# arloan/OpticalImageProcessor

Hardware: AMD Instinct MI355X
Metric: Mpix/s end-to-end RRC+stitch on 30000x100000x4 strip; % HBM roofline (higher is better)
Workload: dtype u16 rasters; fp64 RRC/maps, f32 bicubic and FFT; 1 GPU; default action (--do-rrc4pan): PAN 30000x100000 + MSS 4x(7500x25000) per GPU; RRC + 5x10x4 inter-band phase correlations (16000x3000 FFT) + polyfit + bicubic align to 16UC4; width=30000, pan_lines_per_gpu=100000, parallelism=rowblock1, backend=rccl, inputs=resident in HBM

## Files before the change

### opticalimageprocessor_amd/csrc/phasecorr.hip

```cpp
#include "oip_corrgeom.h"
#include "oip_fft.h"
#include "oip_fft_dev.h"
#include "oip_internal.h"

#include <cfloat>
#include <cmath>

namespace {

constexpr int kBlock = 256;

__global__ __launch_bounds__(kBlock) void window_u16_to_f32_kernel(const uint16_t *__restrict__ img, size_t pitch,
                                                                   long row0, int col0, int rows, int cols,
                                                                   float *__restrict__ out)
{
    long i = (long)blockIdx.x * kBlock + threadIdx.x;
    const long n = (long)rows * cols;
    const long stride = (long)gridDim.x * kBlock;
    for (; i < n; i += stride) {
        long y = i / cols;
        int x = (int)(i - y * cols);
        out[i] = (float)img[(size_t)(row0 + y) * pitch + col0 + x];
    }
}
// ... 298 lines not shown
    commit(threadIdx.x);
    long s1 = n1, s2 = n2;
    __syncthreads();
    for (; ky <= half; ky += gridDim.x) {
        int tid = threadIdx.x;
        asm volatile("" : "+v"(tid));
        const bool pair = s1 != s2;
        const int kn = ky + gridDim.x;
        const bool more = kn <= half;
        if (more) {
            n1 = (long)ypos[kn] * P;
            n2 = (long)ypos[M - kn] * P;
            fetch(tid);
        }
        __builtin_amdgcn_sched_barrier(0);
        row_stages<ALL, F, NT, NARR, Rs...>(buf, tw, tid);
#pragma unroll 1
        for (int it = 0; it < NIT; ++it) {
            const int kx = tid + it * NT;
            if (kx >= N) continue;
            const int nkx = kx ? N - kx : 0;
            const bool edge_col = (kx == 0) || (2 * kx == N);
            const bool real_bin = edge_col && (ky == 0 || 2 * ky == M);
            const float2 zk0 = buf[2 * kx], zm0 = buf[2 * nkx + 1];
            const float2 A = spec_of(0, zk0, zm0);
            float2 y0, y0m, y1 = make_float2(0.f, 0.f), y1m = make_float2(0.f, 0.f);
            {
                const float2 C = cross_power_bin_fast(A, spec_of(1, zk0, zm0), real_bin, edge_col);
                y0 = C;
                y0m = make_float2(C.x, -C.y);
            }
            if (NARR == 3) {
                const float2 zk1 = buf[2 * F + 2 * kx], zm1 = buf[2 * F + 2 * nkx + 1];
                const float2 zk2 = buf[4 * F + 2 * kx], zm2 = buf[4 * F + 2 * nkx + 1];
                float2 C = cross_power_bin_fast(A, spec_of(0, zk1, zm1), real_bin, edge_col);
                y0.x -= C.y; y0.y += C.x; y0m.x += C.y; y0m.y += C.x;
                C = cross_power_bin_fast(A, spec_of(1, zk1, zm1), real_bin, edge_col);
                y1 = C;
                y1m = make_float2(C.x, -C.y);
                const float2 B3 = fj.last_part ? spec_of(1, zk2, zm2) : spec_of(0, zk2, zm2);
                C = cross_power_bin_fast(A, B3, real_bin, edge_col);
                y1.x -= C.y; y1.y += C.x; y1m.x += C.y; y1m.y += C.x;
            }
            buf[2 * kx] = make_float2(y0.x, -y0.y);
            buf[2 * nkx + 1] = pair ? make_float2(y0m.x, -y0m.y) : make_float2(0.f, 0.f);
            if (NOUT == 2) {
                buf[2 * F + 2 * kx] = make_float2(y1.x, -y1.y);
                buf[2 * F + 2 * nkx + 1] = pair ? make_float2(y1m.x, -y1m.y) : make_float2(0.f, 0.f);
            }
        }
        __syncthreads();
        asm volatile("" : "+v"(tid));
        row_stages<ALL, F, NT, NOUT, Rs...>(buf, tw, tid);
        if (!ALL && NOUT == 1) __syncthreads();
        float4 ya[NOUT][NIT2], yb[NOUT][NIT2];
#pragma unroll
        for (int o = 0; o < NOUT; ++o) {
#pragma unroll
            for (int it = 0; it < NIT2; ++it) {
                const int q = tid + it * NT;
                if (q < N / 2) {
                    const float4 u = buf4[o * F + 2 * q], v = buf4[o * F + 2 * q + 1];
                    ya[o][it] = make_float4(u.x, -u.y, v.x, -v.y);
                    yb[o][it] = make_float4(u.z, -u.w, v.z, -v.w);
                }
            }
        }
        __syncthreads();
        if (more) commit(tid);
        __builtin_amdgcn_sched_barrier(0);
        const long o1 = s1, o2 = s2;
        s1 = n1; s2 = n2;
#pragma unroll
        for (int o = 0; o < NOUT; ++o) {
            float2 *out = fj.out[o];
#pragma unroll
            for (int it = 0; it < NIT2; ++it) {
                const int q = tid + it * NT;
                if (q < N / 2) {
                    *reinterpret_cast<float4 *>(out + o1 + 2 * q) = ya[o][it];
                    if (pair) *reinterpret_cast<float4 *>(out + o2 + 2 * q) = yb[o][it];
                }
            }
        }
        __syncthreads();
    }
}

struct UpRowsJob {
    const float2 *zp;
    const float2 *zn;
    long zn_stride;
    int Pn;
    float2 *out[4];
    const float2 *xtab;
    int nout;
    const float2 *vtab;
    const uint2 *raw16;
    const int *ypos_s;
    int m;
    float *bound;
    int win_hi, win_lo;
};

__device__ __forceinline__ float2 cmulj(float2 a, float2 b)
{
    oipfft::oip_v2f t, r;
    asm("v_pk_mul_f32 %0, %1, %2 op_sel_hi:[0,1]" : "=v"(t) : "v"(oipfft::to_v(a)), "v"(oipfft::to_v(b)));
    asm("v_pk_fma_f32 %0, %1, %2, %3 op_sel:[1,1,0] op_sel_hi:[1,0,1] neg_hi:[1,0,0]" : "=v"(r) : "v"(oipfft::to_v(a)), "v"(oipfft::to_v(b)), "v"(t));
    return oipfft::to_f2(r);
}
__device__ __forceinline__ float2 cfma(float2 a, float2 b, float2 acc)
{
    oipfft::oip_v2f t, r;
    asm("v_pk_fma_f32 %0, %1, %2, %3 op_sel_hi:[0,1,1]" : "=v"(t) : "v"(oipfft::to_v(a)), "v"(oipfft::to_v(b)), "v"(oipfft::to_v(acc)));
    asm("v_pk_fma_f32 %0, %1, %2, %3 op_sel:[1,1,0] op_sel_hi:[1,0,1] neg_lo:[1,0,0]" : "=v"(r) : "v"(oipfft::to_v(a)), "v"(oipfft::to_v(b)), "v"(t));
    return oipfft::to_f2(r);
}
__device__ __forceinline__ float2 cfmaj(float2 a, float2 b, float2 acc)
{
    oipfft::oip_v2f t, r;
    asm("v_pk_fma_f32 %0, %1, %2, %3 op_sel_hi:[0,1,1]" : "=v"(t) : "v"(oipfft::to_v(a)), "v"(oipfft::to_v(b)), "v"(oipfft::to_v(acc)));
    asm("v_pk_fma_f32 %0, %1, %2, %3 op_sel:[1,1,0] op_sel_hi:[1,0,1] neg_hi:[1,0,0]" : "=v"(r) : "v"(oipfft::to_v(a)), "v"(oipfft::to_v(b)), "v"(t));
    return oipfft::to_f2(r);
}

__device__ __forceinline__ float2 spec2_of(int part, float2 zk, float2 zm)
{
    if (part == 0) return make_float2(zk.x + zm.x, zk.y - zm.y);
    return make_float2(zk.y + zm.y, zm.x - zk.x);
}
__device__ __forceinline__ float2 sfma(float s, float2 v, float2 acc)
{
    OIP_FFT_FMA
    return make_float2(acc.x + s * v.x, acc.y + s * v.y);
}

template <int NT, bool VEXP, bool WIN>
__global__ __launch_bounds__(NT) void corr_rows_up_kernel(UpRowsJob fj, int M, int P, const int *__restrict__ ypos,
                                                          const float2 *__restrict__ twF, const float2 *__restrict__ twS)
{
    constexpr int F = 3000, S = F / 4;
    constexpr int TWF = oipfft::TwTable<F, 25, 15, 8>::value(), TWS = oipfft::TwTable<S, 25, 15, 2>::value();
    constexpr int NB = (F / 2 + 1 + NT - 1) / NT;
    __shared__ __align__(16) float2 buf[2 * 2 * F + 4 * 2 * S];
    __shared__ float2 tw[TWF], tws[TWS];
    __shared__ float2 edge[4][2][4];
    __shared__ float2 edgeA[2][2];
    __shared__ float2 edgeT[2][5];
    float2 *bufN = buf + 4 * F;
    float4 *buf4 = reinterpret_cast<float4 *>(buf), *buf4N = reinterpret_cast<float4 *>(bufN);
    const int half = M / 2;
    int ky = blockIdx.x;
    if (ky > half) return;
    for (int i = threadIdx.x; i < TWF; i += NT) tw[i] = twF[i];
    for (int i = threadIdx.x; i < TWS; i += NT) tws[i] = twS[i];
    if (threadIdx.x < 10) edgeT[threadIdx.x / 5][threadIdx.x % 5] = fj.xtab[(threadIdx.x % 5) * F + (threadIdx.x / 5) * (F / 2)];
    float2 H[NB], G[NB][4];
    auto load_tables = [&](int tid) {
#pragma unroll
        for (int r = 0; r < NB; ++r) {
            int kx = tid + NT * r;
            kx = kx <= F / 2 ? kx : 0;
            H[r] = fj.xtab[kx];
#pragma unroll
            for (int j = 0; j < 4; ++j) G[r][j] = fj.xtab[(1 + j) * F + kx];
        }
    };
    constexpr int NIT2 = (F / 2 + NT - 1) / NT;
    constexpr int NQ = 4 * (S / 2);
    constexpr int NITN = (NQ + NT - 1) / NT;
    float4 la[NIT2], lb[NIT2], na[NITN], nb[NITN];
    long n1 = ypos[ky], n2 = ypos[ky ? M - ky : 0];
    auto narrow_row = [&](int k, long full) { return VEXP ? (long)fj.ypos_s[k % fj.m] : full; };
    long m1 = narrow_row(ky, n1), m2 = narrow_row(ky ? M - ky : 0, n2);
    int kyc = ky;
    float2 vt[5];
    uint2 rawreg[NITN][4];
    auto fetch_narrow = [&](int tid) {
        if (VEXP) {
#pragma unroll
            for (int r = 0; r < 5; ++r) vt[r] = fj.vtab[r * M + kyc];
#pragma unroll
            for (int it = 0; it < NITN; ++it) {
                int q = tid + it * NT;
                q = q < NQ ? q : NQ - 1;
#pragma unroll
                for (int r = 0; r < 4; ++r) rawreg[it][r] = fj.raw16[(long)r * NQ + q];
            }
        }
#pragma unroll
        for (int it = 0; it < NITN; ++it) {
            int q = tid + it * NT;
            q = q < NQ ? q : NQ - 1;
            const int a = q / (S / 2), i = q - a * (S / 2);
            const float2 *z = fj.zn + a * fj.zn_stride + 2 * i;
            na[it] = *reinterpret_cast<const float4 *>(z + m1 * fj.Pn);
            nb[it] = *reinterpret_cast<const float4 *>(z + m2 * fj.Pn);
        }
    };
    auto fetch = [&](int tid) {
#pragma unroll
        for (int it = 0; it < NIT2; ++it) {
            int q = tid + it * NT;
            q = q < F / 2 ? q : F / 2 - 1;
            la[it] = *reinterpret_cast<const float4 *>(fj.zp + n1 * P + 2 * q);
            lb[it] = *reinterpret_cast<const float4 *>(fj.zp + n2 * P + 2 * q);
        }
        if (!VEXP) fetch_narrow(tid);
    };
    auto commit = [&](int tid) {
        if (VEXP) fetch_narrow(tid);
#pragma unroll
        for (int it = 0; it < NIT2; ++it) line_pair_commit<F>(buf4, 0, la[it], lb[it], tid + it * NT);
#pragma unroll
        for (int it = 0; it < NITN; ++it) {
            const int q = tid + it * NT;
            if (q < NQ) {
                const int a = q / (S / 2), i = q - a * (S / 2);
                if (VEXP) {
                    const float2 hv = vt[0];
                    float2 x0 = oipfft::cmul(hv, make_float2(na[it].x, na[it].y)), x1 = oipfft::cmul(hv, make_float2(na[it].z, na[it].w));
                    float2 y0 = cmulj(hv, make_float2(nb[it].x, nb[it].y)), y1 = cmulj(hv, make_float2(nb[it].z, nb[it].w));
#pragma unroll
                    for (int r = 0; r < 4; ++r) {
                        const float2 gv = vt[1 + r];
                        const uint2 u = rawreg[it][r];
                        const float2 w0 = make_float2((float)(u.x & 0xffffu), (float)(u.x >> 16)), w1 = make_float2((float)(u.y & 0xffffu), (float)(u.y >> 16));
                        x0 = cfma(gv, w0, x0); x1 = cfma(gv, w1, x1);
                        y0 = cfmaj(gv, w0, y0); y1 = cfmaj(gv, w1, y1);
                    }
                    na[it] = make_float4(x0.x, x0.y, x1.x, x1.y);
                    nb[it] = make_float4(y0.x, y0.y, y1.x, y1.y);
                }
                buf4N[a * S + 2 * i] = make_float4(na[it].x, na[it].y, nb[it].x, nb[it].y);
                buf4N[a * S + 2 * i + 1] = make_float4(na[it].z, na[it].w, nb[it].z, nb[it].w);
                if (i == 0 || i == S / 2 - 1) {
                    const int j = i ? 2 : 0;
                    edge[a][0][j] = make_float2(na[it].x, na[it].y); edge[a][0][j + 1] = make_float2(na[it].z, na[it].w);
                    edge[a][1][j] = make_float2(nb[it].x, nb[it].y); edge[a][1][j + 1] = make_float2(nb[it].z, nb[it].w);
                }
            }
        }
    };
    fetch(threadIdx.x);
    commit(threadIdx.x);
    long s1 = n1, s2 = n2;
    __syncthreads();
    bool first = true;
    char *const brow = reinterpret_cast<char *>(fj.bound + (long)blockIdx.x * 4 * P);
    for (; ky <= half; ky += gridDim.x) {
        int tid = threadIdx.x;
        asm volatile("" : "+v"(tid));
        const bool pair = s1 != s2;
        const int kn = ky + gridDim.x;
        const bool more = kn <= half;
        if (first) load_tables(tid);
        first = false;
        __builtin_amdgcn_sched_barrier(0);
        oipfft::StagesDual3<F, 1, S, 4, NT, 25, 15, 8, 2>::run(buf, tw, bufN, tws, tid);
        float2 Aa[2 * NB], Ab[2 * NB];
#pragma unroll
        for (int r = 0; r < NB; ++r) {
            const int kx = tid + NT * r, nkx = kx ? F - kx : 0;
            if (kx <= F / 2) {
                const float2 zk = buf[2 * kx], zm = buf[2 * nkx + 1];
                Aa[2 * r] = spec_of(0, zk, zm);
                Ab[2 * r] = spec_of(1, zk, zm);
                const float2 zk2 = buf[2 * nkx], zm2 = buf[2 * kx + 1];
                Aa[2 * r + 1] = spec_of(0, zk2, zm2);
                Ab[2 * r + 1] = spec_of(1, zk2, zm2);
                if (kx == 0 || 2 * kx == F) { edgeA[kx ? 1 : 0][0] = Aa[2 * r]; edgeA[kx ? 1 : 0][1] = Ab[2 * r]; }
            }
        }
        auto xround = [&](int o0, const float2 (&A)[2 * NB]) {
#pragma unroll
            for (int h = 0; h < 2; ++h) {
                const float2 *zn = bufN + (o0 + h) * 2 * S;
                float2 e0[4], e1[4];
#pragma unroll
                for (int j = 0; j < 4; ++j) { e0[j] = edge[o0 + h][0][j]; e1[j] = edge[o0 + h][1][j]; }
                float2 *ob = buf + h * 2 * F;
#pragma unroll
                for (int r = 0; r < NB; ++r) {
                    const int kx = tid + NT * r, nkx = kx ? F - kx : 0;
                    if (kx > F / 2) continue;
                    const int c = kx % S, cm = c ? S - c : 0;
                    float2 S0 = make_float2(0.f, 0.f), T0 = S0, S1 = S0, T1 = S0;
#pragma unroll
                    for (int j = 0; j < 4; ++j) {
                        S0 = sfma(G[r][j].x, e0[j], S0); T0 = sfma(G[r][j].y, e0[j], T0);
                        S1 = sfma(G[r][j].x, e1[j], S1); T1 = sfma(G[r][j].y, e1[j], T1);
                    }
                    {
                        const float2 Z0 = oipfft::csub_rot(oipfft::cadd(oipfft::cmul(H[r], zn[2 * c]), S0), T0);
                        const float2 Z1 = oipfft::cadd_rot(oipfft::cadd(cmulj(H[r], zn[2 * cm + 1]), S1), T1);
                        const float2 C1 = cross_power_bin_fast(A[2 * r], spec2_of(0, Z0, Z1), false, false);
                        const float2 C2 = cross_power_bin_fast(A[2 * r], spec2_of(1, Z0, Z1), false, false);
                        ob[2 * kx] = make_float2(C1.x - C2.y, -(C1.y + C2.x));
                        ob[2 * nkx + 1] = pair ? make_float2(C1.x + C2.y, -(C2.x - C1.y)) : make_float2(0.f, 0.f);
                    }
                    if (kx != 0 && 2 * kx != F) {
                        const float2 Z0 = oipfft::cadd_rot(oipfft::cadd(cmulj(H[r], zn[2 * cm]), S0), T0);
                        const float2 Z1 = oipfft::csub_rot(oipfft::cadd(oipfft::cmul(H[r], zn[2 * c + 1]), S1), T1);
                        const float2 C1 = cross_power_bin_fast(A[2 * r + 1], spec2_of(0, Z0, Z1), false, false);
                        const float2 C2 = cross_power_bin_fast(A[2 * r + 1], spec2_of(1, Z0, Z1), false, false);
                        ob[2 * nkx] = make_float2(C1.x - C2.y, -(C1.y + C2.x));
                        ob[2 * kx + 1] = pair ? make_float2(C1.x + C2.y, -(C2.x - C1.y)) : make_float2(0.f, 0.f);
                    }
                    __builtin_amdgcn_sched_barrier(0);
                }
            }
#pragma unroll 1
            for (int r = 0; r < NB; ++r) {
                const int kx = tid + NT * r;
                if (kx != 0 && 2 * kx != F) continue;
                const bool real_bin = ky == 0 || 2 * ky == M;
                const float2 Ae = edgeA[kx ? 1 : 0][o0 ? 1 : 0];
                float2 He = edgeT[kx ? 1 : 0][0], Ge[4];
#pragma unroll
                for (int j = 0; j < 4; ++j) Ge[j] = edgeT[kx ? 1 : 0][1 + j];
#pragma unroll 1
                for (int h = 0; h < 2; ++h) {
                    const float2 *zn = bufN + (o0 + h) * 2 * S;
                    float2 Z0 = oipfft::cmul(He, zn[0]), Z1 = cmulj(He, zn[1]);
#pragma unroll
                    for (int j = 0; j < 4; ++j) { Z0 = cfma(Ge[j], edge[o0 + h][0][j], Z0); Z1 = cfmaj(Ge[j], edge[o0 + h][1][j], Z1); }
                    const float2 C1 = cross_power_bin(Ae, spec2_of(0, Z0, Z1), real_bin, true);
                    const float2 C2 = cross_power_bin(Ae, spec2_of(1, Z0, Z1), real_bin, true);
                    float2 *ob = buf + h * 2 * F;
                    ob[2 * kx] = make_float2(C1.x - C2.y, -(C1.y + C2.x));
                    ob[2 * kx + 1] = pair ? make_float2(C1.x + C2.y, -(C2.x - C1.y)) : make_float2(0.f, 0.f);
                }
            }
        };
        float4 ya[2][NIT2], yb[2][NIT2];
        auto finish = [&]() {
            __syncthreads();
            asm volatile("" : "+v"(tid));
            oipfft::StagesAll<F, NT, 2, 1, 25, 15, 8>::run(buf, tw, tid);
#pragma unroll
            for (int o = 0; o < 2; ++o) {
#pragma unroll
                for (int it = 0; it < NIT2; ++it) line_pair_read_conj<F>(ya[o][it], yb[o][it], buf4, o * F, tid + it * NT);
            }
            __syncthreads();
        };
        auto store = [&](int o0) {
#pragma unroll
            for (int o = 0; o < 2; ++o) {
                float2 *out = fj.out[o0 + o];
#pragma unroll
                for (int it = 0; it < NIT2; ++it) {
                    const int q = tid + it * NT;
                    if (!WIN || q < fj.win_hi || q >= fj.win_lo) line_pair_store<F>(out, s1 * P, s2 * P, pair, ya[o][it], yb[o][it], q);
                }
            }
        };
        auto bound_add = [&](int o0) {
            int tb = tid;
            asm volatile("" : "+v"(tb));
#pragma unroll
            for (int o = 0; o < 2; ++o) {
#pragma unroll
                for (int it = 0; it < NIT2; ++it) {
                    const int q = tb + it * NT;
                    if (q < F / 2) {
                        const float4 a = ya[o][it], b = yb[o][it];
                        float2 s = make_float2(fabsf(a.x) + fabsf(a.y), fabsf(a.z) + fabsf(a.w));
                        if (pair) { s.x += fabsf(b.x) + fabsf(b.y); s.y += fabsf(b.z) + fabsf(b.w); }
                        float *bp = reinterpret_cast<float *>(brow + (unsigned)((o0 + o) * P + 2 * q) * 4u);
                        unsafeAtomicAdd(bp, s.x);
                        unsafeAtomicAdd(bp + 1, s.y);
                    }
                }
            }
        };
        xround(0, Aa);
        finish();
        if (fj.nout == 4) load_tables(tid);
        __builtin_amdgcn_sched_barrier(0);
        store(0);
        __builtin_amdgcn_sched_barrier(0);
        bound_add(0);
        if (fj.nout == 4) xround(2, Ab);
        __builtin_amdgcn_sched_barrier(0);
        if (more) {
            n1 = oip_sload_i32(ypos, kn);
            n2 = oip_sload_i32(ypos, M - kn);
            m1 = VEXP ? (long)oip_sload_i32(fj.ypos_s, kn % fj.m) : n1;
            m2 = VEXP ? (long)oip_sload_i32(fj.ypos_s, (M - kn) % fj.m) : n2;
            kyc = kn;
            fetch(tid);
        }
        __builtin_amdgcn_sched_barrier(0);
        if (fj.nout == 4) finish();
        if (more) commit(tid);
        __builtin_amdgcn_sched_barrier(0);
        if (more) load_tables(tid);
        __builtin_amdgcn_sched_barrier(0);
        if (fj.nout == 4) {
            store(2);
            __builtin_amdgcn_sched_barrier(0);
            bound_add(2);
        }
        s1 = n1; s2 = n2;
        __syncthreads();
    }
}

struct VRowsJob {
    const float2 *zp;
    const float2 *zn;
    long zn_stride;
    int Pn;
    float2 *out[4];
    int nout;
    const float2 *vtab;
    const float2 *raw;
    const int *ypos_s;
    int m;
};

template <int F, int NT, int... Rs>
__global__ __launch_bounds__(NT, 2 * NT / 256) void corr_rows_v_kernel(VRowsJob fj, int a0, int part, int M, int P, const int *__restrict__ ypos,
                                                                      const float2 *__restrict__ twF)
{
    constexpr int TWN = oipfft::TwTable<F, Rs...>::value();
    constexpr int N = F, NARR = 3, NB = 2;
    constexpr int NIT = (N + NT - 1) / NT;
    static_assert(N % 2 == 0, "two points per lane");
    constexpr int NIT2 = (N / 2 + NT - 1) / NT;
    constexpr int NQ = NB * (N / 2);
    constexpr int NITN = (NQ + NT - 1) / NT;
    __shared__ __align__(16) float2 buf[NARR * 2 * F];
    __shared__ float2 tw[TWN];
    float4 *buf4 = reinterpret_cast<float4 *>(buf);
    const int half = M / 2;
    int ky = blockIdx.x;
    if (ky > half) return;
    for (int i = threadIdx.x; i < TWN; i += NT) tw[i] = twF[i];
    float4 la[NIT2], lb[NIT2], na[NITN], nb[NITN];
    float2 vt[5];
    long n1 = ypos[ky], n2 = ypos[ky ? M - ky : 0];
    long m1 = fj.ypos_s[ky % fj.m], m2 = fj.ypos_s[(ky ? M - ky : 0) % fj.m];
    int kyc = ky;
    const float2 *zn = fj.zn + (long)a0 * fj.zn_stride;
    const float2 *raw = fj.raw + (long)a0 * fj.zn_stride;
    auto fetch = [&](int tid) {
#pragma unroll
        for (int it = 0; it < NIT2; ++it) {
            int q = tid + it * NT;
            q = q < N / 2 ? q : N / 2 - 1;
            la[it] = *reinterpret_cast<const float4 *>(fj.zp + n1 * P + 2 * q);
            lb[it] = *reinterpret_cast<const float4 *>(fj.zp + n2 * P + 2 * q);
        }
#pragma unroll
        for (int it = 0; it < NITN; ++it) {
            int q = tid + it * NT;
            q = q < NQ ? q : NQ - 1;
            const int a = q / (N / 2), i = q - a * (N / 2);
            const float2 *z = zn + a * fj.zn_stride + 2 * i;
            na[it] = *reinterpret_cast<const float4 *>(z + m1 * fj.Pn);
            nb[it] = *reinterpret_cast<const float4 *>(z + m2 * fj.Pn);
        }
#pragma unroll
        for (int r = 0; r < 5; ++r) vt[r] = fj.vtab[r * M + kyc];
    };
    auto commit = [&](int tid) {
#pragma unroll
        for (int it = 0; it < NIT2; ++it) line_pair_commit<N>(buf4, 0, la[it], lb[it], tid + it * NT);
#pragma unroll
        for (int it = 0; it < NITN; ++it) {
            const int q = tid + it * NT;
            if (q >= NQ) continue;
            const int a = q / (N / 2), i = q - a * (N / 2);
            const float2 hv = vt[0];
            float2 x0 = oipfft::cmul(hv, make_float2(na[it].x, na[it].y)), x1 = oipfft::cmul(hv, make_float2(na[it].z, na[it].w));
            float2 y0 = cmulj(hv, make_float2(nb[it].x, nb[it].y)), y1 = cmulj(hv, make_float2(nb[it].z, nb[it].w));
#pragma unroll
            for (int r = 0; r < 4; ++r) {
                const float4 rw = *reinterpret_cast<const float4 *>(raw + ((long)r * 4 + a) * fj.zn_stride + 2 * i);
                const float2 gv = vt[1 + r];
                const float2 w0 = make_float2(rw.x, rw.y), w1 = make_float2(rw.z, rw.w);
                x0 = cfma(gv, w0, x0); x1 = cfma(gv, w1, x1);
                y0 = cfmaj(gv, w0, y0); y1 = cfmaj(gv, w1, y1);
            }
            buf4[(1 + a) * F + 2 * i] = make_float4(x0.x, x0.y, y0.x, y0.y);
            buf4[(1 + a) * F + 2 * i + 1] = make_float4(x1.x, x1.y, y1.x, y1.y);
        }
    };
    fetch(threadIdx.x);
    commit(threadIdx.x);
    long s1 = n1, s2 = n2;
    __syncthreads();
    for (; ky <= half; ky += gridDim.x) {
        int tid = threadIdx.x;
        asm volatile("" : "+v"(tid));
        const bool pair = s1 != s2;
        const int kn = ky + gridDim.x;
        const bool more = kn <= half;
        if (more) {
            n1 = ypos[kn];
            n2 = ypos[M - kn];
            m1 = fj.ypos_s[kn % fj.m];
            m2 = fj.ypos_s[(M - kn) % fj.m];
            kyc = kn;
            fetch(tid);
        }
        __builtin_amdgcn_sched_barrier(0);
        oipfft::StagesPipe<F, NT, NARR, 1, Rs...>::run(buf, tw, tid);
#pragma unroll 1
        for (int it = 0; it < NIT; ++it) {
            const int kx = tid + it * NT;
            if (kx >= N) continue;
            const int nkx = kx ? N - kx : 0;
            const bool edge_col = (kx == 0) || (2 * kx == N);
            const bool real_bin = edge_col && (ky == 0 || 2 * ky == M);
            const float2 A = spec_of(part, buf[2 * kx], buf[2 * nkx + 1]);
#pragma unroll
            for (int a = 0; a < NB; ++a) {
                float2 *b = buf + (1 + a) * 2 * F;
                const float2 zk = b[2 * kx], zm = b[2 * nkx + 1];
                const float2 C1 = cross_power_bin_fast(A, spec_of(0, zk, zm), real_bin, edge_col);
                const float2 C2 = cross_power_bin_fast(A, spec_of(1, zk, zm), real_bin, edge_col);
                b[2 * kx] = make_float2(C1.x - C2.y, -(C1.y + C2.x));
                b[2 * nkx + 1] = pair ? make_float2(C1.x + C2.y, -(C2.x - C1.y)) : make_float2(0.f, 0.f);
            }
        }
        __syncthreads();
        asm volatile("" : "+v"(tid));
        oipfft::StagesPipe<F, NT, NB, 1, Rs...>::run(buf + 2 * F, tw, tid);
        float4 ya[NB][NIT2], yb[NB][NIT2];
#pragma unroll
        for (int o = 0; o < NB; ++o) {
#pragma unroll
            for (int it = 0; it < NIT2; ++it) line_pair_read_conj<N>(ya[o][it], yb[o][it], buf4, (1 + o) * F, tid + it * NT);
        }
        __syncthreads();
        if (more) commit(tid);
        __builtin_amdgcn_sched_barrier(0);
#pragma unroll
        for (int o = 0; o < NB; ++o) {
            float2 *out = fj.out[a0 + o];
#pragma unroll
            for (int it = 0; it < NIT2; ++it) line_pair_store<N>(out, s1 * P, s2 * P, pair, ya[o][it], yb[o][it], tid + it * NT);
        }
        s1 = n1; s2 = n2;
        __syncthreads();
    }
}

struct HPackJob {
    const uint16_t *bx[4], *by[4];
    long pitch[4];
};
__global__ __launch_bounds__(128) void hpack_bands_kernel(HPackJob job, int m, int n, int cols, int stride, int Pn, const int *__restrict__ xofs,
                                                          const float4 *__restrict__ alpha, float2 *__restrict__ z, float2 *__restrict__ raw)
{
    const int x = blockIdx.x * 128 + threadIdx.x;
    const int a = blockIdx.z;
// ... 685 lines not shown
    double *const res[1] = {d_result};
    return peak_windows(ctx, pl, w, y, res, 1, 1);
}

int correlate_four(oip_ctx *ctx, const OipFft2dPlan *pl, const PcWork &w, const FusedRow *rk, float2 *zp, float2 *zq,
                   float2 *zl, int last_part, double *d_results )
{
    const SpecRef sa[4] = {{zp, 0}, {zp, 0}, {zp, 0}, {zp, 0}};
    const SpecRef sb[4] = {{zp, 1}, {zq, 0}, {zq, 1}, {zl, last_part}};
    float2 *const y[2] = {w.y[0], w.y[1]};
    int rc;
    if ((rc = xpower_stage(ctx, pl, rk, sa, sb, 4, y))) return rc;
    if ((rc = inverse_to_slots(ctx, pl, w, w.y[0], rk != nullptr, 0))) return rc;
    if ((rc = inverse_to_slots(ctx, pl, w, w.y[1], rk != nullptr, 1))) return rc;
    double *const res[2] = {d_results, d_results + 6};
    return peak_windows(ctx, pl, w, y, res, 2, 2);
}

int correlate_one_to_four(oip_ctx *ctx, const OipFft2dPlan *pl, const PcWork &w, RealSrc a, const RealSrc b[4],
                          int rows, int cols, double *d_results , const HTaps *vt)
{
    const FusedRow *rk = row_stage(pl);
    const bool skip = rk != nullptr;
    int rc;
    if ((rc = forward_packed(ctx, pl, w.z[0], a, b[0], rows, cols, skip, vt))) return rc;
    if ((rc = forward_packed(ctx, pl, w.z[1], b[1], b[2], rows, cols, skip, vt))) return rc;
    if ((rc = forward_packed(ctx, pl, w.z[2], b[3], src_none(), rows, cols, skip, vt))) return rc;
    return correlate_four(ctx, pl, w, rk, w.z[0], w.z[1], w.z[2], 0, d_results);
}

int correlate_two_units(oip_ctx *ctx, const OipFft2dPlan *pl, const PcWork &w, RealSrc aA, const RealSrc bA[4], RealSrc aB,
                        const RealSrc bB[4], int rows, int cols, double *d_resA , double *d_resB, const HTaps *vt)
{
    const FusedRow *rk = row_stage(pl);
    const bool skip = rk != nullptr;
    int rc;
    if ((rc = forward_packed(ctx, pl, w.z[0], aA, bA[0], rows, cols, skip, vt))) return rc;
    if ((rc = forward_packed(ctx, pl, w.z[1], bA[1], bA[2], rows, cols, skip, vt))) return rc;
    if ((rc = forward_packed(ctx, pl, w.z[2], aB, bB[0], rows, cols, skip, vt))) return rc;
    if ((rc = forward_packed(ctx, pl, w.z[3], bB[1], bB[2], rows, cols, skip, vt))) return rc;
    if ((rc = forward_packed(ctx, pl, w.z[4], bA[3], bB[3], rows, cols, skip, vt))) return rc;
    if ((rc = correlate_four(ctx, pl, w, rk, w.z[0], w.z[1], w.z[4], 0, d_resA))) return rc;
    return correlate_four(ctx, pl, w, rk, w.z[2], w.z[3], w.z[4], 1, d_resB);
}

struct IbUnit {
    const uint16_t *pan;
    long pan_pitch;
    const uint16_t *band[OIP_MSS_BANDS];
    long band_pitch;
};

struct UpPath {
    const OipFft2dPlan *narrow;
    const OipFft2dPlan *small;
    const float2 *xtab, *vtab;
    bool vonly;
};

struct BandPackJob {
    const uint16_t *bx[4], *by[4];
    long pitch[4];
};
template <bool PAIRS>
__global__ __launch_bounds__(128) void pack_bands_kernel(BandPackJob job, int m, int n, int Pn, float2 *__restrict__ z, unsigned *__restrict__ raw16)
{
    constexpr int W = PAIRS ? 2 : 1;
    const int p = W * (blockIdx.x * 128 + threadIdx.x);
    const int a = blockIdx.z;
    if (p >= n) return;
    const uint16_t *bx = job.bx[a] + p, *by = job.by[a] + p;
    const long pitch = job.pitch[a];
#pragma unroll 4
    for (int y = blockIdx.y; y < m; y += gridDim.y) {
        const int r = y < 2 ? y : (y >= m - 2 ? y - (m - 4) : -1);
        if (PAIRS) {
            const unsigned ux = *reinterpret_cast<const unsigned *>(bx + y * pitch), uy = *reinterpret_cast<const unsigned *>(by + y * pitch);
            *reinterpret_cast<float4 *>(z + (long)y * Pn + a * n + p) =
                make_float4((float)(ux & 0xffffu), (float)(uy & 0xffffu), (float)(ux >> 16), (float)(uy >> 16));
            if (r >= 0) *reinterpret_cast<uint2 *>(raw16 + ((long)r * 4 + a) * n + p) = make_uint2((ux & 0xffffu) | (uy << 16), (ux >> 16) | (uy & 0xffff0000u));
        } else {
            const unsigned ux = bx[y * pitch], uy = by[y * pitch];
            z[(long)y * Pn + a * n + p] = make_float2((float)ux, (float)uy);
            if (r >= 0) raw16[((long)r * 4 + a) * n + p] = ux | (uy << 16);
        }
    }
}

int correlate_units_up(oip_ctx *ctx, const OipFft2dPlan *pl, const UpPath &up, const PcWork &w, RealSrc aA, RealSrc aB, const RealSrc *v ,
                       const IbUnit *const *units, int nunits, int rows, int cols, int band_rows, int band_cols, double *d_resA, double *d_resB,
                       int win_r = -1, int *d_miss = nullptr)
{
    int rc;
    if ((rc = forward_packed(ctx, pl, w.z[0], aA, nunits > 1 ? aB : src_none(), rows, cols, true))) return rc;
    const int narr = 2 * nunits;
    long zn_stride;
    int Pn;
    const int *ypos_s = nullptr;
    unsigned *raw = nullptr;
    if (up.vtab) {
        Pn = up.small->P;
        zn_stride = band_cols;
        raw = reinterpret_cast<unsigned *>(w.z[1] + (long)up.small->M * Pn);
        BandPackJob bj;
        for (int a = 0; a < 4; ++a) {
            const IbUnit *u = units[(a < narr ? a : 0) / 2];
            bj.bx[a] = u->band[2 * (a & 1)]; bj.by[a] = u->band[2 * (a & 1) + 1]; bj.pitch[a] = u->band_pitch;
        }
        {
            OipProfScope prof(ctx, "pack_bands_kernel");
            bool pairs = (band_cols & 1) == 0 && (Pn & 1) == 0;
            for (int a = 0; a < 4; ++a)
                pairs = pairs && (bj.pitch[a] & 1) == 0 && ((size_t)bj.bx[a] & 3) == 0 && ((size_t)bj.by[a] & 3) == 0;
            const int gy = band_rows < 128 ? band_rows : 128;
            if (pairs)
                hipLaunchKernelGGL(pack_bands_kernel<true>, dim3((band_cols / 2 + 127) / 128, gy, 4), dim3(128), 0, ctx->stream, bj, band_rows, band_cols, Pn,
                                   w.z[1], raw);
            else
                hipLaunchKernelGGL(pack_bands_kernel<false>, dim3((band_cols + 127) / 128, gy, 4), dim3(128), 0, ctx->stream, bj, band_rows, band_cols, Pn,
                                   w.z[1], raw);
            OIP_HIP(ctx, hipGetLastError());
        }
        ctx->prof_tag = "_band";
        rc = oip_fft2d_exec(ctx, up.small, w.z[1], 0, nullptr, 1);
        ctx->prof_tag = nullptr;
        if (rc) return rc;
        ypos_s = up.small->d_ypos;
    } else {
        Pn = up.narrow->P;
        zn_stride = (long)up.narrow->M * Pn;
        ctx->prof_tag = "_quarter";
        for (int a = 0; a < narr && !rc; ++a)
            rc = forward_packed(ctx, up.narrow, w.z[1] + a * zn_stride, src_f32(v[2 * a].v), src_f32(v[2 * a + 1].v), rows, band_cols, true);
        ctx->prof_tag = nullptr;
        if (rc) return rc;
    }
    const float2 *twF, *twS;
    if ((rc = oip_fft_table(ctx, 3000, &twF)) || (rc = oip_fft_table(ctx, 750, &twS))) return rc;
    UpRowsJob fj;
    memset(&fj, 0, sizeof fj);
    fj.zp = w.z[0];
    fj.zn = w.z[1];
    fj.zn_stride = zn_stride;
    fj.Pn = Pn;
    for (int o = 0; o < 4; ++o) fj.out[o] = w.y[o];
    fj.xtab = up.xtab;
    fj.nout = narr;
    fj.vtab = up.vtab;
    fj.raw16 = reinterpret_cast<const uint2 *>(raw);
    fj.ypos_s = ypos_s;
    fj.m = band_rows;
    fj.bound = w.prune.bound;
    if (!fj.bound) return oip_fail(ctx, OIP_E_RUNTIME, "correlate_units_up: no storage for the column bounds");
    OIP_HIP(ctx, hipMemsetAsync(fj.bound, 0, sizeof(float) * (size_t)w.prune.groups * 4 * pl->P, ctx->stream));
    PruneWork pw = w.prune;
    const char *pe = getenv("OIP_PEAK_PRUNE");
    const int full = pe && atoi(pe) == 0 ? 1 : 0;
    if (full || !up.vtab || !rows_window_fits(pw, win_r) || !d_miss) win_r = -1;
    pw.win_r = win_r;
    pw.miss = d_miss;
    if (win_r >= 0) {
        fj.win_hi = ((win_r + 1) << pw.vshift) / 2;
        fj.win_lo = ((pw.T - win_r) << pw.vshift) / 2;
    }
    {
        const char *pz = getenv("OIP_ROWS_WINDOW_POISON");
        if (pz && atoi(pz) > 0)
            for (int o = 0; o < narr; ++o) OIP_HIP(ctx, hipMemsetAsync(w.y[o], 0xff, sizeof(float2) * (size_t)pl->M * pl->P, ctx->stream));
    }
    {
        OipProfScope prof(ctx, "corr_rows_up_kernel");
        const long grid = w.prune.groups;
        const dim3 g((unsigned)grid);
        auto k = up.vtab ? (win_r >= 0 ? corr_rows_up_kernel<512, true, true> : corr_rows_up_kernel<512, true, false>)
                         : corr_rows_up_kernel<512, false, false>;
        hipLaunchKernelGGL(k, g, dim3(512), 0, ctx->stream, fj, pl->M, pl->P, pl->d_ypos, twF, twS);
        OIP_HIP(ctx, hipGetLastError());
    }
    double *res[4];
    for (int o = 0; o < narr; ++o) res[o] = (o < 2 ? d_resA : d_resB) + 6 * (o & 1);
    if (!pw.tiles) {
        for (int o = 0; o < narr; ++o)
            if ((rc = inverse_to_slots(ctx, pl, w, w.y[o], true, o))) return rc;
        return peak_windows(ctx, pl, w, w.y, res, narr, 2);
    }
    if (!ctx->d_prune_stats) {
        OIP_HIP(ctx, hipMalloc((void **)&ctx->d_prune_stats, 2 * sizeof(unsigned long long)));
        OIP_HIP(ctx, hipMemsetAsync(ctx->d_prune_stats, 0, 2 * sizeof(unsigned long long), ctx->stream));
    }
    {
        OipProfScope prof(ctx, "col_sel_first_kernel");
        hipLaunchKernelGGL(col_sel_first_kernel, dim3((pl->N + kSelCols - 1) / kSelCols, narr), dim3(kSelThreads), 0, ctx->stream, pw, pl->P, pl->N, full);
        OIP_HIP(ctx, hipGetLastError());
    }
    OipColList cl;
    memset(&cl, 0, sizeof cl);
    for (int o = 0; o < 4; ++o) cl.data[o] = w.y[o < narr ? o : 0];
    cl.stride = pw.T;
    cl.narr = narr;
    cl.slots = w.slots;
    for (int phase = 0; phase < 2; ++phase) {
        if (phase == 1) {
            OipProfScope prof(ctx, "col_sel_second_kernel");
            hipLaunchKernelGGL(col_sel_second_kernel, dim3(narr), dim3(kPeakSlots), 0, ctx->stream, pw, w.slots, ctx->d_prune_stats);
            OIP_HIP(ctx, hipGetLastError());
            if (full) break;
        }
        for (int kind = 0; kind < 2; ++kind) {
            cl.count = pw.count + (phase * 2 + kind) * 4;
            cl.tiles = pw.tiles + (long)(phase * 2 + kind) * 4 * pw.T;
            if (kind == 1) {
                if ((rc = oip_fft_col_list_pass(ctx, pl, 0, cl, true, "col_sel_peak"))) return rc;
                continue;
            }
            for (int i = pl->n_y - 1; i >= 1; --i) {
                char name[32];
                snprintf(name, sizeof name, "col_sel_F%d", pl->passes[i].F);
                if ((rc = oip_fft_col_list_pass(ctx, pl, i, cl, false, name))) return rc;
            }
        }
    }
    return peak_windows(ctx, pl, w, w.y, res, narr, 2);
}

int correlate_units_vup(oip_ctx *ctx, const OipFft2dPlan *pl, const UpPath &up, const PcWork &w, const OipResizeTab *tab, RealSrc aA, RealSrc aB,
                        const IbUnit *const *units, int nunits, int rows, int cols, int band_rows, int band_cols, double *d_resA, double *d_resB)
{
    int rc;
    if ((rc = forward_packed(ctx, pl, w.z[0], aA, nunits > 1 ? aB : src_none(), rows, cols, true))) return rc;
    const int narr = 2 * nunits;
    const int N = pl->N, Pn = up.small->P;
    float2 *zn = w.z[1];
    float2 *raw = reinterpret_cast<float2 *>(w.fsmall);
    if ((long)up.small->M * Pn > (long)pl->M * pl->P) return oip_fail(ctx, OIP_E_RUNTIME, "correlate_units_vup: band array exceeds its slot");
    HPackJob hj;
    for (int a = 0; a < 4; ++a) {
        const IbUnit *u = units[(a < narr ? a : 0) / 2];
        hj.bx[a] = u->band[2 * (a & 1)]; hj.by[a] = u->band[2 * (a & 1) + 1]; hj.pitch[a] = u->band_pitch;
    }
    {
        OipProfScope prof(ctx, "hpack_bands_kernel");
        const int gy = band_rows < 256 ? band_rows : 256;
        hipLaunchKernelGGL(hpack_bands_kernel, dim3((N + 127) / 128, gy, 4), dim3(128), 0, ctx->stream, hj, band_rows, band_cols, cols, N, Pn, tab->d_xofs,
                           reinterpret_cast<const float4 *>(tab->d_alpha), zn, raw);
        OIP_HIP(ctx, hipGetLastError());
    }
    ctx->prof_tag = "_band";
    rc = oip_fft2d_exec(ctx, up.small, zn, 0, nullptr, 1);
    ctx->prof_tag = nullptr;
    if (rc) return rc;
    const float2 *twF;
    if ((rc = oip_fft_table(ctx, N, &twF))) return rc;
    VRowsJob fj;
    memset(&fj, 0, sizeof fj);
    fj.zp = w.z[0];
    fj.zn = zn;
    fj.zn_stride = N;
    fj.Pn = Pn;
    for (int o = 0; o < 4; ++o) fj.out[o] = w.y[o];
    fj.nout = narr;
    fj.vtab = up.vtab;
    fj.raw = raw;
    fj.ypos_s = up.small->d_ypos;
    fj.m = band_rows;
    {
        OipProfScope prof(ctx, "corr_rows_v_kernel");
        long grid = 2L * ctx->cu_count;
        if (grid > pl->M / 2 + 1) grid = pl->M / 2 + 1;
        if (N != 1250) return oip_fail(ctx, OIP_E_RUNTIME, "correlate_units_vup: no row stage for %d-point rows", N);
        for (int u = 0; u < nunits; ++u)
            hipLaunchKernelGGL((corr_rows_v_kernel<1250, 512, 5, 5, 5, 5, 2>), dim3((unsigned)grid), dim3(512), 0, ctx->stream, fj, 2 * u, u, pl->M, pl->P,
                               pl->d_ypos, twF);
        OIP_HIP(ctx, hipGetLastError());
    }
    double *res[4];
    for (int o = 0; o < narr; ++o) {
        res[o] = (o < 2 ? d_resA : d_resB) + 6 * (o & 1);
        if ((rc = inverse_to_slots(ctx, pl, w, w.y[o], true, o))) return rc;
    }
    return peak_windows(ctx, pl, w, w.y, res, narr, 2);
}

int fetch_results(oip_ctx *ctx, int count, double *host_out, int nflags = 0, int *flags_out = nullptr)
{
    ctx->prof_chain = nullptr;
    OIP_HIP(ctx, hipMemcpyAsync(ctx->h_small, ctx->d_small, sizeof(double) * count + sizeof(int) * nflags, hipMemcpyDeviceToHost, ctx->stream));
    OIP_HIP(ctx, hipStreamSynchronize(ctx->stream));
    memcpy(host_out, ctx->h_small, sizeof(double) * count);
    if (nflags) memcpy(flags_out, (const char *)ctx->h_small + sizeof(double) * count, sizeof(int) * nflags);
    return OIP_OK;
}

}

extern "C" int oip_window_u16_to_f32(oip_ctx *ctx, const uint16_t *d_img, size_t pitch, long row0, int col0, int rows,
                                     int cols, float *d_out)
{
    OIP_CHECK_CTX(ctx);
    if (!d_img || !d_out || rows <= 0 || cols <= 0 || row0 < 0 || col0 < 0 || (size_t)(col0 + cols) > pitch)
        return oip_fail(ctx, OIP_E_INVALID, "oip_window_u16_to_f32: bad argument");
    return launch_window(ctx, d_img, pitch, row0, col0, rows, cols, d_out);
}

extern "C" int oip_resize_cubic_f32(oip_ctx *ctx, const float *d_src, int sw, int sh, float *d_dst, int dw, int dh)
{
    OIP_CHECK_CTX(ctx);
    if (!d_src || !d_dst || sw <= 0 || sh <= 0 || dw <= 0 || dh <= 0 || dh > 65535)
// ... 289 lines not shown
```

Measured before the change: 88740 Mpix/s.

## Accumulate column bounds in registers and store once per block

After: 93560 Mpix/s, median of 6. 5.4% higher.

```diff
diff --git a/opticalimageprocessor_amd/csrc/phasecorr.hip b/opticalimageprocessor_amd/csrc/phasecorr.hip
--- a/opticalimageprocessor_amd/csrc/phasecorr.hip
+++ b/opticalimageprocessor_amd/csrc/phasecorr.hip
@@ -474,7 +474,25 @@
     float4 *buf4 = reinterpret_cast<float4 *>(buf), *buf4N = reinterpret_cast<float4 *>(bufN);
     const int half = M / 2;
     int ky = blockIdx.x;
-    if (ky > half) return;
+    constexpr int NIT2 = (F / 2 + NT - 1) / NT;
+    float2 acc[4][NIT2];
+#pragma unroll
+    for (int o = 0; o < 4; ++o) {
+#pragma unroll
+        for (int it = 0; it < NIT2; ++it) acc[o][it] = make_float2(0.f, 0.f);
+    }
+    auto write_bounds = [&]() {
+        float *brow = fj.bound + (long)blockIdx.x * 4 * P;
+#pragma unroll
+        for (int o = 0; o < 4; ++o) {
+#pragma unroll
+            for (int it = 0; it < NIT2; ++it) {
+                const int q = threadIdx.x + it * NT;
+                if (q < F / 2) *reinterpret_cast<float2 *>(brow + o * P + 2 * q) = acc[o][it];
+            }
+        }
+    };
+    if (ky > half) { write_bounds(); return; }
     for (int i = threadIdx.x; i < TWF; i += NT) tw[i] = twF[i];
     for (int i = threadIdx.x; i < TWS; i += NT) tws[i] = twS[i];
     if (threadIdx.x < 10) edgeT[threadIdx.x / 5][threadIdx.x % 5] = fj.xtab[(threadIdx.x % 5) * F + (threadIdx.x / 5) * (F / 2)];
@@ -489,7 +507,6 @@
             for (int j = 0; j < 4; ++j) G[r][j] = fj.xtab[(1 + j) * F + kx];
         }
     };
-    constexpr int NIT2 = (F / 2 + NT - 1) / NT;
     constexpr int NQ = 4 * (S / 2);
     constexpr int NITN = (NQ + NT - 1) / NT;
     float4 la[NIT2], lb[NIT2], na[NITN], nb[NITN];
@@ -569,16 +586,13 @@
     commit(threadIdx.x);
     long s1 = n1, s2 = n2;
     __syncthreads();
-    bool first = true;
-    char *const brow = reinterpret_cast<char *>(fj.bound + (long)blockIdx.x * 4 * P);
+    load_tables(threadIdx.x);
     for (; ky <= half; ky += gridDim.x) {
         int tid = threadIdx.x;
         asm volatile("" : "+v"(tid));
         const bool pair = s1 != s2;
         const int kn = ky + gridDim.x;
         const bool more = kn <= half;
-        if (first) load_tables(tid);
-        first = false;
         __builtin_amdgcn_sched_barrier(0);
         oipfft::StagesDual3<F, 1, S, 4, NT, 25, 15, 8, 2>::run(buf, tw, bufN, tws, tid);
         float2 Aa[2 * NB], Ab[2 * NB];
@@ -656,55 +670,32 @@
                 }
             }
         };
-        float4 ya[2][NIT2], yb[2][NIT2];
-        auto finish = [&]() {
+        auto finish = [&](int o0) {
             __syncthreads();
             asm volatile("" : "+v"(tid));
             oipfft::StagesAll<F, NT, 2, 1, 25, 15, 8>::run(buf, tw, tid);
 #pragma unroll
             for (int o = 0; o < 2; ++o) {
-#pragma unroll
-                for (int it = 0; it < NIT2; ++it) line_pair_read_conj<F>(ya[o][it], yb[o][it], buf4, o * F, tid + it * NT);
+                float2 *out = fj.out[o0 + o];
+#pragma unroll
+                for (int it = 0; it < NIT2; ++it) {
+                    const int q = tid + it * NT;
+                    if (q < F / 2) {
+                        float4 a, b;
+                        line_pair_read_conj<F>(a, b, buf4, o * F, q);
+                        if (!WIN || q < fj.win_hi || q >= fj.win_lo) line_pair_store<F>(out, s1 * P, s2 * P, pair, a, b, q);
+                        float2 s = make_float2(fabsf(a.x) + fabsf(a.y), fabsf(a.z) + fabsf(a.w));
+                        if (pair) { s.x += fabsf(b.x) + fabsf(b.y); s.y += fabsf(b.z) + fabsf(b.w); }
+                        acc[o0 + o][it].x += s.x;
+                        acc[o0 + o][it].y += s.y;
+                    }
+                }
             }
             __syncthreads();
         };
-        auto store = [&](int o0) {
-#pragma unroll
-            for (int o = 0; o < 2; ++o) {
-                float2 *out = fj.out[o0 + o];
-#pragma unroll
-                for (int it = 0; it < NIT2; ++it) {
-                    const int q = tid + it * NT;
-                    if (!WIN || q < fj.win_hi || q >= fj.win_lo) line_pair_store<F>(out, s1 * P, s2 * P, pair, ya[o][it], yb[o][it], q);
-                }
-            }
-        };
-        auto bound_add = [&](int o0) {
-            int tb = tid;
-            asm volatile("" : "+v"(tb));
-#pragma unroll
-            for (int o = 0; o < 2; ++o) {
-#pragma unroll
-                for (int it = 0; it < NIT2; ++it) {
-                    const int q = tb + it * NT;
-                    if (q < F / 2) {
-                        const float4 a = ya[o][it], b = yb[o][it];
-                        float2 s = make_float2(fabsf(a.x) + fabsf(a.y), fabsf(a.z) + fabsf(a.w));
-                        if (pair) { s.x += fabsf(b.x) + fabsf(b.y); s.y += fabsf(b.z) + fabsf(b.w); }
-                        float *bp = reinterpret_cast<float *>(brow + (unsigned)((o0 + o) * P + 2 * q) * 4u);
-                        unsafeAtomicAdd(bp, s.x);
-                        unsafeAtomicAdd(bp + 1, s.y);
-                    }
-                }
-            }
-        };
         xround(0, Aa);
-        finish();
-        if (fj.nout == 4) load_tables(tid);
+        finish(0);
         __builtin_amdgcn_sched_barrier(0);
-        store(0);
-        __builtin_amdgcn_sched_barrier(0);
-        bound_add(0);
         if (fj.nout == 4) xround(2, Ab);
         __builtin_amdgcn_sched_barrier(0);
         if (more) {
@@ -716,19 +707,12 @@
             fetch(tid);
         }
         __builtin_amdgcn_sched_barrier(0);
-        if (fj.nout == 4) finish();
+        if (fj.nout == 4) finish(2);
         if (more) commit(tid);
-        __builtin_amdgcn_sched_barrier(0);
-        if (more) load_tables(tid);
-        __builtin_amdgcn_sched_barrier(0);
-        if (fj.nout == 4) {
-            store(2);
-            __builtin_amdgcn_sched_barrier(0);
-            bound_add(2);
-        }
         s1 = n1; s2 = n2;
         __syncthreads();
     }
+    write_bounds();
 }
 
 struct VRowsJob {
@@ -1720,7 +1704,7 @@
     fj.m = band_rows;
     fj.bound = w.prune.bound;
     if (!fj.bound) return oip_fail(ctx, OIP_E_RUNTIME, "correlate_units_up: no storage for the column bounds");
-    OIP_HIP(ctx, hipMemsetAsync(fj.bound, 0, sizeof(float) * (size_t)w.prune.groups * 4 * pl->P, ctx->stream));
+    if (pl->P & 1) return oip_fail(ctx, OIP_E_RUNTIME, "correlate_units_up: odd row pitch %d", pl->P);
     PruneWork pw = w.prune;
     const char *pe = getenv("OIP_PEAK_PRUNE");
     const int full = pe && atoi(pe) == 0 ? 1 : 0;
```
